# QizhiPei/FABind

Measured on AMD Instinct MI355X. Metric: complexes/sec fwd+bwd (1500p/40l nodes), full IaBNet on the whole graph (pocket model + 4-layer complex model + distance-map head on all nodes / pairs) with the pocket-cls + pocket-centre + coord + distmap + distmap-by-coords + distill losses (BASELINE configs[2] read literally), higher is better.
Workload: dtype bf16

## Files before the change

fabind_amd/_lib.py:

```python
import ctypes
import os

import torch

from . import config as _cfg

_HERE = os.path.dirname(os.path.abspath(__file__))
LIB_PATH = _cfg.knob("FABIND_LIB") or os.path.join(_HERE, "libfabind_hip.so")

ABI_VERSION = 19
DT_F32, DT_BF16 = 0, 1
ACT_NONE, ACT_SILU, ACT_RELU, ACT_SIGMOID, ACT_STORED_DERIV = 0, 1, 2, 3, 4
GEMM_FAM_NT_F32, GEMM_FAM_NT_F32_BF16, GEMM_FAM_NT_BF16, GEMM_FAM_GLDS, GEMM_FAM_PIPE, GEMM_FAM_X3, GEMM_FAM_X3_PRO, GEMM_FAM_PERSIST = range(8)

_vp, _i, _f, _l = ctypes.c_void_p, ctypes.c_int, ctypes.c_float, ctypes.c_long


class GemmArgs(ctypes.Structure):
    _fields_ = [(n, _vp) for n in ("A", "A2", "W", "C", "bias", "R", "r_index", "dotvec", "dot_out", "aux", "groups", "C2")] + \
               [(n, _i) for n in ("M", "N", "K", "K1", "lda", "lda2", "ldw", "ldc", "ldr", "ldaux", "dot_ld",
                                  "a_dtype", "w_dtype", "c_dtype", "aux_dtype", "act_pro", "act_epi", "dact_epi",
                                  "accumulate", "store_preact", "n_groups", "max_m", "max_n", "groups_ext", "epi_fast", "k_splits")] + \
               [("alpha", _f), ("p_drop", _f), ("drop_seed", ctypes.c_uint)] + \
               [(n, _vp) for n in ("row_mu", "row_rs", "col_c", "C16")] + [("ldc16", _i), ("split3", _i), ("r_dtype", _i), ("c2_bf16", _i)]
# ... 103 lines not shown
    "fabind_rowdot_bwd": [_vp, _i, _vp, _i, _vp, _i, _i, _i, _vp, _vp, _vp, _i, _vp],
    "fabind_edge_geom_bwd": [_vp, _vp, _vp, _vp, _vp, _vp, _vp, _vp, _vp, _vp, _i, _i, _i, _vp, _vp, _vp, _vp],
    "fabind_gcl_pre_bwd": [_vp, _i, _i, _vp, _vp, _i, _vp, _vp, _vp, _i, _vp],
    "fabind_gather_dact": [_vp, _i, _vp, _vp, _i, _i, _vp, _i, _i, _i, _vp],
    "fabind_coord_update_bwd": [_vp, _vp, _vp, _i, _i, _f, _vp, _vp, _vp, _vp],
    "fabind_cross_attn_bwd": [_vp, _i, _vp, _i, _vp, _i, _i, _i, _vp, _i, _i, _i, _f, _vp, _vp, _vp, _vp, _vp, _vp, _vp,
                              _vp, _vp, _vp],
    "fabind_pair_bias_cat": [_vp, _i, _vp, _i, _i, _i, _vp, _i, _vp, _i, _vp, _vp, _i, _vp, _i, _vp, _vp],
    "fabind_batched_transpose_pad": [_vp, _i, _vp, _i, _i, _i, _i, _vp, _vp],
    "fabind_node_chain_fwd": [_vp, _i, _vp, _i, _vp, _vp, _vp, _vp, _vp, _vp, _i, _i, _vp, _i, _vp, _i, _vp, _i, _i, _i, _vp],
    "fabind_node_chain_x3_fwd": [_vp, _i, _vp, _i, _vp, _vp, _vp, _vp, _vp, _vp, _vp, _vp, _vp, _vp, _i, _i, _vp, _i, _vp, _i, _vp, _i, _vp, _i, _vp, _i,
                                 _i, _i, _vp],
    "fabind_rows_hadamard_bwd": [_vp, _i, _i, _vp, _i, _i, _vp, _vp, _vp, _i, _vp, _i, _vp],
    "fabind_pair_hadamard_bwd_grid": [_vp, _i, _i, _vp, _i, _i, _vp, _vp, _vp, _vp, _i, _vp, _i, _vp],
    "fabind_pair_hadamard_bwd_rows": [_vp, _i, _i, _vp, _i, _i, _vp, _i, _i, _vp, _vp, _vp, _vp, _i, _vp, _i, _vp, _i, _vp],
    "fabind_pair_hadamard_bwd": [_vp, _i, _i, _vp, _vp, _i, _i, _vp, _vp, _i, _i, _vp, _vp, _i, _vp, _vp, _i, _vp, _vp, _i,
                                 _vp],
    "fabind_inter_attn_bwd": [_vp, _i, _vp, _i, _i, _vp, _vp, _vp, _vp, _vp, _vp, _vp, _vp, _vp, _vp, _vp, _vp, _f, _i,
                              _vp, _vp, _vp, _vp, _vp, _vp, _vp, _vp, _vp, _vp, _i, _vp],
    "fabind_inter_attn_bwd_rows": [_vp, _i, _vp, _i, _i, _vp, _vp, _vp, _vp, _vp, _vp, _vp, _vp, _vp, _vp, _vp, _vp, _f, _i,
                                   _vp, _vp, _vp, _vp, _vp, _vp, _vp, _vp, _vp, _vp, _i, _vp, _i, _i, _vp],
    "fabind_las_step_bwd": [_vp, _vp, _vp, _vp, _vp, _vp, _vp, _vp, _i, _i, _f, _f, _vp, _vp, _vp],
    "fabind_pair_bias_bwd": [_vp, _i, _vp, _i, _i, _vp, _vp, _i, _i, _i, _vp, _vp, _vp, _vp, _vp],
    "fabind_pair_bias_btcat": [_vp, _i, _vp, _vp, _vp, _i, _i, _i, _vp, _i, _i, _vp],
    "fabind_pair_bias_finish": [_vp, _vp, _i, _i, _vp, _vp, _i, _vp, _vp, _l, _vp],
    "fabind_pack_frag_multi": [_vp, _vp, _i, _vp],
    "fabind_lower_bound": [_vp, _i, _vp, _i, _vp, _vp],
    "fabind_pocket_center_fwd": [_vp, _vp, _vp, _vp, _i, _i, _f, _i, _vp, _vp, _vp],
    "fabind_pocket_center_bwd": [_vp, _vp, _vp, _vp, _i, _i, _f, _vp, _vp, _vp, _vp, _vp],
    "fabind_pair_dist_fwd": [_vp, _i, _i, _vp, _vp, _f, _f, _f, _vp, _vp],
    "fabind_pair_dist_bwd": [_vp, _i, _i, _vp, _vp, _vp, _f, _f, _f, _vp, _vp, _vp],
    "fabind_block_hadamard_fwd": [_vp, _i, _i, _vp, _i, _vp, _i, _i, _vp, _i, _vp],
    "fabind_block_hadamard_bwd": [_vp, _i, _i, _vp, _i, _vp, _i, _vp, _i, _i, _vp, _i, _i, _vp, _vp, _i, _vp, _i, _vp],
    "fabind_loss_fwd": [_vp, _vp, _l, _vp, _vp, _vp, _l, _vp, _vp, _i, _vp, _l, _vp, _vp, _l, _f, _f, _f, _f, _f, _f, _vp, _vp, _vp, _vp, _vp, _vp],
    "fabind_loss_bwd": [_vp, _vp, _l, _vp, _vp, _vp, _l, _vp, _vp, _i, _l, _vp, _vp, _l, _f, _f, _f, _f, _f, _f, _vp, _vp, _vp,
                        _vp, _vp, _vp, _vp, _vp, _vp],
    "fabind_layernorm_fwd": [_vp, _vp, _vp, _f, _i, _i, _vp, _vp, _vp, _vp],
    "fabind_layernorm_bwd": [_vp, _vp, _vp, _vp, _vp, _i, _i, _vp, _vp, _vp, _vp],
}

_lib = None


def load():
    global _lib
    if _lib is not None:
        return _lib
    if not os.path.exists(LIB_PATH):
        raise RuntimeError(
            "fabind_amd: %s is missing -- build it with `python -m fabind_amd.build` (hipcc, gfx950). "
            "There is no CPU/eager fallback for the hot path." % LIB_PATH)
    lib = ctypes.CDLL(LIB_PATH)
    lib.fabind_last_error.restype = ctypes.c_char_p
    lib.fabind_abi_version.restype = ctypes.c_int
    got = lib.fabind_abi_version()
    if got != ABI_VERSION:
        raise RuntimeError("fabind_amd: %s has ABI version %d, this binding needs %d -- rebuild with `python -m fabind_amd.build`"
                           % (LIB_PATH, got, ABI_VERSION))
    lib.fabind_sizeof_args.argtypes, lib.fabind_sizeof_args.restype = [ctypes.c_int], ctypes.c_int
    lib.fabind_cross_attn_bwd_scratch.argtypes, lib.fabind_cross_attn_bwd_scratch.restype = [_i, _i, _i], ctypes.c_long
    lib.fabind_pair_bias_cat_parts.argtypes, lib.fabind_pair_bias_cat_parts.restype = [_i, _i], ctypes.c_long
    lib.fabind_cross_attn_fused_bwd_scratch.argtypes, lib.fabind_cross_attn_fused_bwd_scratch.restype = [_i, _i, _i, _i, _i], ctypes.c_long
    lib.fabind_cross_attn_fused_bwd_parts.argtypes, lib.fabind_cross_attn_fused_bwd_parts.restype = [_i, _i], ctypes.c_int
    lib.fabind_pair_bias_finish_parts.argtypes, lib.fabind_pair_bias_finish_parts.restype = [_i], ctypes.c_int
    lib.fabind_loss_blocks.argtypes, lib.fabind_loss_blocks.restype = [_l, _l, _l], ctypes.c_int
    for nm in ("fabind_pair_block_tile", "fabind_pair_block_chunk"):
# ... 58 lines not shown
```

fabind_amd/build.py:

```python
import os
import subprocess
import sys

HERE = os.path.dirname(os.path.abspath(__file__))
CSRC = os.path.join(HERE, "csrc")
INCLUDE = os.path.join(os.path.dirname(HERE), "include")
LIB = os.path.join(HERE, "libfabind_hip.so")
SOURCES = ["capi.hip", "gemm.hip", "graph.hip", "gcl.hip", "fused_edge.hip", "fused_edge_fwd2.hip", "fused_edge_fwd3.hip", "fused_edge_bwd3.hip", "fused_edge_bwd4.hip", "pair_fused.hip", "attn.hip", "inter_attn_rows.hip", "attn_mfma.hip", "norm.hip", "bwd.hip", "post_optim.hip", "node_chain.hip", "heads.hip", "symmetry.hip", "optim.hip"]
HIPCC = os.environ.get("HIPCC", "/opt/rocm/bin/hipcc")
FLAGS = ["--offload-arch=gfx950", "-O3", "-std=c++17", "-fPIC", "-Wno-comment", "-I" + INCLUDE, "-I" + CSRC]


def _stale(out, deps):
    if not os.path.exists(out):
        return True
    t = os.path.getmtime(out)
    return any(os.path.getmtime(d) > t for d in deps)


def build(force=False, verbose=True):
    objs = []
    hdrs = [os.path.join(CSRC, "common.h"), os.path.join(CSRC, "fused_common.h"), os.path.join(INCLUDE, "fabind_hip.h")]
    procs = []
    for src in SOURCES:
        sp = os.path.join(CSRC, src)
        if not os.path.exists(sp):
            raise RuntimeError("fabind_amd.build: source %s is missing" % sp)
        obj = os.path.join(CSRC, src.replace(".hip", ".o"))
        objs.append(obj)
        if force or _stale(obj, [sp] + hdrs):
            cmd = [HIPCC] + FLAGS + ["-c", sp, "-o", obj]
            if verbose:
                print(" ".join(cmd), flush=True)
            procs.append((src, subprocess.Popen(cmd)))
    for src, p in procs:
        if p.wait() != 0:
            raise RuntimeError("hipcc failed on " + src)
    if force or procs or _stale(LIB, objs):
        cmd = [HIPCC, "--offload-arch=gfx950", "-shared", "-fPIC", "-o", LIB] + objs
        if verbose:
            print(" ".join(cmd), flush=True)
# ... 7 lines not shown
```

fabind_amd/models/model.py:

```python
import random

import torch
import torch.nn as nn
import torch.nn.functional as F
from torch.nn import Linear

from .. import kernels as K
from .. import ops
from ..utils.utils import get_keepNode_tensor, gumbel_softmax_no_random
from .att_model import EfficientMCAttModel


class Transition_diff_out_dim(nn.Module):

    def __init__(self, embedding_channels=256, out_channels=256, n=4):
        super().__init__()
        self.layernorm = nn.LayerNorm(embedding_channels)
        self.linear1 = Linear(embedding_channels, n * embedding_channels)
        self.linear2 = Linear(n * embedding_channels, out_channels)
        torch.nn.init.xavier_uniform_(self.linear1.weight, gain=0.001)
        torch.nn.init.xavier_uniform_(self.linear2.weight, gain=0.001)

    def forward(self, z):
        shp = z.shape
# ... 252 lines not shown
        start = _offsets(reps)
        j = torch.arange(pi.shape[0], device=dev) - start[pi]
        ci = _offsets(ncnt)[pocket_batch][pi] + j
        kn = torch.stack([kcnt, ncnt]).tolist()
        return _Pairs(pi, ci, ops.PairBlocks(kn[0], kn[1], dev))

    def _complex_and_heads(self, data, g, plan=None):
        scale = self.coordinate_scale
        cb = data['compound'].batch
        if plan:
            Xn, Xl, cidx, pidx = plan['Xn'], plan['Xl'], plan['cidx'], plan['pidx']
        else:
            Xn = self.normalize_coord(g['X'].unsqueeze(-2)).float()
            Xl = self.normalize_coord(g['XL'].unsqueeze(-2)).float()
            seg1 = g['segment'].bool() if not g['segment'].is_floating_point() else g['segment'] > 0.5
            cidx = torch.nonzero(~seg1 & ~g['is_global']).squeeze(1)
            pidx = torch.nonzero(seg1 & ~g['is_global']).squeeze(1)
        Xo, Ho = self.complex_model(Xn, g['H'], batch_id=g['batch'], segment_id=g['segment'], mask=g['mask'],
                                    is_global=g['is_global'], compound_edge_index=g['c2c'], LAS_edge_index=g['LAS'],
                                    batched_complex_coord_LAS=Xl, LAS_mask=None)
        coords_n = ops.take_unique_rows(Xo, cidx).squeeze(-2)
        return Ho, cidx, pidx, coords_n

    def _dist_heads(self, data, g, Ho, cidx, pidx, coords_n):
        cb = data['compound'].batch
        pairs = g.get('pairs')
        if pairs is None:
            B = int(cb[-1].item()) + 1
            pairs = self._pair_lists(g['pocket_batch'], cb, torch.bincount(g['pocket_batch'], minlength=B), torch.bincount(cb, minlength=B))
        pi, ci = pairs
        ln = ops.layernorm(ops.take_unique_rows(Ho, torch.cat([pidx, cidx])), self.layernorm.weight, self.layernorm.bias, self.layernorm.eps)
        npk = pidx.shape[0]
        blocks = getattr(pairs, 'blocks', None)
        hd = ops.rows_hadamard(ln, pi, npk + ci, a_sorted=True, blocks=blocks, n_a=npk)
        wd = ops.mm_dtype()
        part = ops.linear_rowdot(hd, self.distmap_mlp[0].weight.to(wd), self.distmap_mlp[0].bias,
                                 self.distmap_mlp[2].weight[0].contiguous(), act_epi=K.ACT_RELU)
        y_pred = (part.sum(1) + self.distmap_mlp[2].bias).sigmoid() * 10
        xp = self.normalize_coord(g['pocket_xyz']).float()
        if blocks is not None and coords_n.is_cuda:
            y_by = ops.pair_dist(xp, coords_n, blocks, scale=self.coordinate_scale, lo=0.0, hi=10.0)
        else:
            y_by = self.unnormalize_coord((xp[pi] - ops.take_rows_few(coords_n, ci)).norm(dim=-1)).clamp(0, 10)
        return y_pred, y_by

    def forward(self, data, stage=1, train=False, plan=None):
        cb = data['compound'].batch
        if plan is not None:
            self._adopt_plan(plan, cb.device)
        if plan is not None:
            keep_idx = plan['keep_idx']
        else:
            keep_idx = torch.nonzero(data['pocket'].keepNode).squeeze(1) if (stage == 1 or self.pocket_pred_model.training) else None
        head = self._pocket_head(data, plan)
        training = self.pocket_pred_model.training
        center = self._soft_center(head['logits'], head['mask'], head['xyz'], noise=training)
        pocket_cls = torch.zeros_like(head['mask'], dtype=data.pocket_idx.dtype)
        pocket_cls[head['pb'], head['loc']] = data.pocket_idx
        if training:
            dist = torch.norm(data.coords_center - center, p=2, dim=-1).mean(dim=-1)
            final_stage = 2 if (dist < self.args.center_dist_threshold and random.random() < self.stage_prob) else 1
        else:
            final_stage = stage
        if final_stage == 2:
            c2 = center
            if self.args.local_eval or (self.args.train_pred_pocket_noise and train):
                c2 = center + self.args.train_pred_pocket_noise * (2 * torch.rand_like(center) - 1)
            g = self._stage2(data, head, c2)
        else:
            cx = data['complex']
            pemb = ops.take_unique_rows(head['p_out'], keep_idx if keep_idx is not None else torch.nonzero(data['pocket'].keepNode).squeeze(1))
# ... 62 lines not shown
```

fabind_amd/ops.py:

```python
import ctypes

import numpy as np
import torch

from . import config as _cfg
from . import kernels as K
from ._lib import GemmArgs, check, dt_code, load, ptr, stream


def act_dtype():
    return torch.float32 if _cfg.fp32_storage() else torch.bfloat16


def mm_dtype():
    return torch.float32 if _cfg.fp32_storage() else torch.bfloat16


def _needs_grad(*ts):
    return torch.is_grad_enabled() and any(torch.is_tensor(t) and t.requires_grad for t in ts)


def needs_grad(*ts):
    return _needs_grad(*ts)

# ... 1828 lines not shown
        ctx.save_for_backward(coords, y_pred, y_by, logits, center, coords_true, dis_map, cls, center_true, out)
        ctx.w, ctx.cls_dt = w, cls_dt
        return loss, terms

    @staticmethod
    def backward(ctx, g_loss, g_terms):
        coords, y_pred, y_by, logits, center, coords_true, dis_map, cls, center_true, out = ctx.saved_tensors
        w = ctx.w
        need = ctx.needs_input_grad
        d = [torch.empty_like(t) if need[i] else None for i, t in enumerate((coords, y_pred, y_by, logits, center))]
        gl = None if g_loss is None else g_loss.contiguous().float()
        gt = None if g_terms is None else g_terms.contiguous().float()
        check(load().fabind_loss_bwd(ptr(coords), ptr(coords_true), coords.numel(), ptr(y_pred), ptr(y_by), ptr(dis_map), y_pred.numel(),
                                     ptr(logits), ptr(cls), ctx.cls_dt, logits.numel(), ptr(center), ptr(center_true), center.numel(),
                                     w['coord'], w['pair'], w['distill'], w['cls'], w['center'], w['delta'], ptr(out), ptr(gl), ptr(gt),
                                     ptr(d[0]), ptr(d[1]), ptr(d[2]), ptr(d[3]), ptr(d[4]), stream()), "fabind_loss_bwd")
        return d[0], d[1], d[2], d[3], d[4], None, None, None, None, None, None


def six_term_loss(coords, y_pred, y_by, logits, center, coords_true, dis_map, pocket_cls, p_mask, center_true, w):
    f = lambda t: t.float().contiguous()
    cls = pocket_cls.contiguous()
    if cls.dtype not in _CLS_DT:
        cls = cls.float()
    m8 = p_mask.contiguous().view(torch.uint8) if p_mask.dtype == torch.bool else p_mask.to(torch.uint8).contiguous()
    w = {k: float(v) for k, v in w.items()}
    loss, terms = _SixTermLoss.apply(f(coords), f(y_pred), f(y_by), f(logits), f(center), f(coords_true), f(dis_map), cls, m8,
                                     f(center_true), w)
    tt = terms.unbind(0)
    return loss, {n: tt[i] for i, n in enumerate(LOSS_TERM_NAMES)}


_PAIRBLOCK = np.dtype([("pair_off", np.int64), ("P", np.int32), ("C", np.int32), ("p_row0", np.int32), ("c_row0", np.int32),
                       ("tile0", np.int32), ("pad", np.int32)])


class PairBlocks:

    def __init__(self, kcnt, ncnt, dev):
        from .param_pack import _upload
        kc, nc = np.asarray(kcnt, dtype=np.int64), np.asarray(ncnt, dtype=np.int64)
        B = kc.shape[0]
        tp, ch = load().fabind_pair_block_tile(), load().fabind_pair_block_chunk()
        tiles = (kc + tp - 1) // tp
        d = np.zeros(B, dtype=_PAIRBLOCK)
        d["pair_off"] = np.cumsum(kc * nc) - kc * nc
        d["P"], d["C"] = kc, nc
        d["p_row0"], d["c_row0"] = np.cumsum(kc) - kc, np.cumsum(nc) - nc
        d["tile0"] = np.cumsum(tiles) - tiles
        self.B, self.n_tiles, self.n_pairs = int(B), int(tiles.sum()), int((kc * nc).sum())
        self.max_C, self.n_prows, self.n_crows = int(nc.max()) if B else 0, int(kc.sum()), int(nc.sum())
        self.nchunk_max = (self.max_C + ch - 1) // ch
        self.chunk = ch
        row_b = np.repeat(np.arange(B, dtype=np.int32), nc)
        raw = np.concatenate([d.view(np.uint8), row_b.view(np.uint8)]) if B else np.zeros(0, dtype=np.uint8)
        self.buf = _upload(raw, dev) if raw.shape[0] else None
        self.desc_bytes = d.view(np.uint8).shape[0]

    def tensors(self):
        return [self.buf] if self.buf is not None else []

    @property
    def desc_ptr(self):
        return self.buf.data_ptr()

    @property
    def row_b_ptr(self):
        return self.buf.data_ptr() + self.desc_bytes


class _PairDist(torch.autograd.Function):
    @staticmethod
    def forward(ctx, xp, xc, blocks, scale, lo, hi):
        y = torch.empty(blocks.n_pairs, dtype=torch.float32, device=xc.device)
        check(load().fabind_pair_dist_fwd(blocks.desc_ptr, blocks.B, blocks.n_tiles, ptr(xp), ptr(xc), scale, lo, hi, ptr(y), stream()),
              "fabind_pair_dist_fwd")
        ctx.save_for_backward(xp, xc)
        ctx.blocks, ctx.k = blocks, (scale, lo, hi)
        return y

    @staticmethod
    def backward(ctx, dy):
        xp, xc = ctx.saved_tensors
        bl = ctx.blocks
        part = torch.empty((bl.B, 8, bl.max_C, 3), dtype=torch.float32, device=xc.device)
        dxc = torch.empty_like(xc)
        check(load().fabind_pair_dist_bwd(bl.desc_ptr, bl.B, bl.max_C, ptr(xp), ptr(xc), ptr(dy.contiguous().float()), ctx.k[0], ctx.k[1],
                                          ctx.k[2], ptr(part), ptr(dxc), stream()), "fabind_pair_dist_bwd")
        return None, dxc, None, None, None, None


def pair_dist(xp, xc, blocks, scale=1.0, lo=0.0, hi=10.0):
    assert not xp.requires_grad, "pair_dist: the pocket coordinates are data"
    xp, xc = xp.float().contiguous(), xc.float().contiguous()
    assert xp.shape[0] == blocks.n_prows and xc.shape[0] == blocks.n_crows
    return _PairDist.apply(xp, xc, blocks, float(scale), float(lo), float(hi))
```

include/fabind_hip.h:

```cpp
#ifndef FABIND_HIP_H
#define FABIND_HIP_H

#include <stdint.h>

#ifdef __cplusplus
extern "C" {
#endif

#ifndef __HIP_PLATFORM_AMD__
typedef struct ihipStream_t* hipStream_t;
#endif

const char* fabind_last_error(void);
#define FABIND_ABI_VERSION 19
int fabind_abi_version(void);
int fabind_sizeof_args(int which);

typedef struct FabindGemmArgs {
    const void* A;
    const void* A2;
    const void* W;
    void* C;
    const float* bias;
    const void* R;
// ... 240 lines not shown
int fabind_las_step(const float* x, const float* x0, const int* las_i, const int* las_j, const int* las_off,
                    const int* node_off, const int* c_cnt, int B, int max_n, float step, float clampv, float* x_out,
                    unsigned char* pass_mask, hipStream_t stream);

int fabind_pocket_center_fwd(const float* logits, const uint8_t* mask, const float* xyz, const float* noise, int B, int L,
                             float tau, int hard, float* center, float* wsum, hipStream_t stream);
int fabind_pocket_center_bwd(const float* logits, const uint8_t* mask, const float* xyz, const float* noise, int B, int L,
                             float tau, const float* center, const float* wsum, const float* dcenter, float* dlogits,
                             hipStream_t stream);

int fabind_loss_blocks(long n_pair, long n_coord, long n_cls);
int fabind_loss_fwd(const float* coords, const float* coords_true, long n_coord, const float* y_pred, const float* y_by,
                    const float* dis_map, long n_pair, const float* logits, const void* cls, int cls_dt, const uint8_t* mask,
                    long n_cls, const float* center, const float* center_true, long n_center, float w_coord, float w_pair,
                    float w_distill, float w_cls, float w_center, float delta, float* part, unsigned* ticket, float* out,
                    float* loss_out, float* terms_out, hipStream_t stream);
int fabind_loss_bwd(const float* coords, const float* coords_true, long n_coord, const float* y_pred, const float* y_by,
                    const float* dis_map, long n_pair, const float* logits, const void* cls, int cls_dt, long n_cls,
                    const float* center, const float* center_true, long n_center, float w_coord, float w_pair, float w_distill,
                    float w_cls, float w_center, float delta, const float* fwd_out, const float* g_loss, const float* g_terms,
                    float* d_coords, float* d_y_pred, float* d_y_by, float* d_logits, float* d_center, hipStream_t stream);

int fabind_pair_block_tile(void);
int fabind_pair_block_chunk(void);
int fabind_pair_dist_fwd(const void* desc, int B, int n_tiles, const float* xp, const float* xc, float scale, float lo, float hi,
                         float* y, hipStream_t stream);
int fabind_pair_dist_bwd(const void* desc, int B, int max_C, const float* xp, const float* xc, const float* dy, float scale, float lo,
                         float hi, float* part, float* dxc, hipStream_t stream);
int fabind_block_hadamard_fwd(const void* desc, int B, int n_tiles, const float* tp, int ldtp, const float* tc, int ldtc, int W, void* out,
                              int ldo, hipStream_t stream);
int fabind_block_hadamard_bwd(const void* desc, int B, int n_tiles, const void* dout, int ldo, const float* tp, int ldtp,
                              const float* tc, int ldtc, int W, const int* row_b, int n_crows, int nchunk_max, float* part,
                              float* dtp, int lddp, float* dtc, int lddc, hipStream_t stream);

int fabind_select_rows(const float* x, const float* z, const uint8_t* mask, int n, int width, float* x_out,
                       hipStream_t stream);

int fabind_row_stats(const void* x, int x_dt, int ldx, float eps, int R, int C, float* mu, float* rs, hipStream_t stream);

int fabind_layernorm_rows(const void* x, int x_dt, int ldx, const float* w, const float* b, float eps, int R, int C, void* y,
                          int y_dt, int ldy, int pad_to, hipStream_t stream);
int fabind_edge_ln_concat(const float* h, int ldh, int H, const int* row, const int* col, const float* rhohat, const float* w,
                          const float* b, float eps, int E, void* y, int y_dt, int ldy, int pad_to, hipStream_t stream);

int fabind_edge_lnfold(const void* AB, int ldab, int Kp, int H, const int* row, const int* col, const float* rho,
                       const float* stat, float eps, const float* w_r, const float* c_r, const float* c_c, const float* dvec,
                       int E, void* out, float p_drop, unsigned seed, hipStream_t stream);
int fabind_edge_lnfold_bwd_blocks(int E);
int fabind_edge_lnfold_bwd(const void* AB, int ldab, int Kp, int H, const int* row, const int* col, const float* rho,
                           const float* stat, float eps, const float* w_r, const float* c_r, const float* c_c,
                           const void* out, const void* dout, int E, float p_drop, void* du, float* es,
                           float* drho, float* part, int n_blocks, hipStream_t stream);

int fabind_inter_coord_fold(const void* P, int ldp, int H, const int* col, const float* rho, const float* stat, float q_w,
                            float eps, const float* u, const float* d, const float* w3, int E, float* s_out, float p_drop,
                            unsigned seed, hipStream_t stream);
int fabind_layernorm_rows_bwd(const void* x, int x_dt, int ldx, const float* w, const void* dy, int dy_dt, int lddy, float eps,
                              int R, int C, void* dx, int dx_dt, int lddx, float* dw_part, float* db_part, int nblk, hipStream_t stream);
int fabind_edge_concat(const float* h, int ldh, int H, const int* row, const int* col, const float* rhohat, int E, void* y,
                       int y_dt, int ldy, int pad_to, hipStream_t stream);
int fabind_layernorm_fwd(const float* x, const float* w, const float* b, float eps, int R, int C, float* y, float* mean,
                         float* rstd, hipStream_t stream);
int fabind_layernorm_bwd(const float* x, const float* w, const float* dy, const float* mean, const float* rstd, int R,
                         int C, float* dx, float* dw_part, float* db_part, hipStream_t stream);

int fabind_add(const float* a, const float* b, float* out, long n, hipStream_t stream);
// ... 93 lines not shown
```

Measured before the change: 527.4.

## Fuse distance-map head hadamard, MLP, relu and rowdot into dedicated kernels

Adds a dist_head forward kernel that builds the pocket×compound Hadamard rows in LDS per 64-row tile, runs the 512×512 MFMA GEMM, and applies bias, ReLU and the w2 dot product in the epilogue. It writes per-pair scores, the bf16 hadamard and pre-activations for backward. A matching backward kernel recomputes ReLU gradients, does the transpose GEMM, and reduces the pocket and compound row gradients plus w2 partials, replacing the separate rows_hadamard and linear_rowdot path. The aim is to cut launches and global round trips over the large pair tensor. In exchange it adds a new zf activation buffer, extra bwd partial reductions and eligibility constraints (H=512, bf16).

```diff
diff --git a/fabind_amd/_lib.py b/fabind_amd/_lib.py
--- a/fabind_amd/_lib.py
+++ b/fabind_amd/_lib.py
@@ -159,6 +159,8 @@
     "fabind_pair_dist_bwd": [_vp, _i, _i, _vp, _vp, _vp, _f, _f, _f, _vp, _vp, _vp],
     "fabind_block_hadamard_fwd": [_vp, _i, _i, _vp, _i, _vp, _i, _i, _vp, _i, _vp],
     "fabind_block_hadamard_bwd": [_vp, _i, _i, _vp, _i, _vp, _i, _vp, _i, _i, _vp, _i, _i, _vp, _vp, _i, _vp, _i, _vp],
+    "fabind_dist_head_fwd": [_vp, _i, _i, _i, _vp, _i, _i, _i, _vp, _vp, _vp, _vp, _vp, _vp, _vp],
+    "fabind_dist_head_bwd": [_vp, _i, _i, _i, _vp, _i, _i, _i, _vp, _vp, _vp, _vp, _vp, _vp, _i, _vp, _i, _vp, _vp, _vp],
     "fabind_loss_fwd": [_vp, _vp, _l, _vp, _vp, _vp, _l, _vp, _vp, _i, _vp, _l, _vp, _vp, _l, _f, _f, _f, _f, _f, _f, _vp, _vp, _vp, _vp, _vp, _vp],
     "fabind_loss_bwd": [_vp, _vp, _l, _vp, _vp, _vp, _l, _vp, _vp, _i, _l, _vp, _vp, _l, _f, _f, _f, _f, _f, _f, _vp, _vp, _vp,
                         _vp, _vp, _vp, _vp, _vp, _vp],
diff --git a/fabind_amd/build.py b/fabind_amd/build.py
--- a/fabind_amd/build.py
+++ b/fabind_amd/build.py
@@ -6,7 +6,7 @@
 CSRC = os.path.join(HERE, "csrc")
 INCLUDE = os.path.join(os.path.dirname(HERE), "include")
 LIB = os.path.join(HERE, "libfabind_hip.so")
-SOURCES = ["capi.hip", "gemm.hip", "graph.hip", "gcl.hip", "fused_edge.hip", "fused_edge_fwd2.hip", "fused_edge_fwd3.hip", "fused_edge_bwd3.hip", "fused_edge_bwd4.hip", "pair_fused.hip", "attn.hip", "inter_attn_rows.hip", "attn_mfma.hip", "norm.hip", "bwd.hip", "post_optim.hip", "node_chain.hip", "heads.hip", "symmetry.hip", "optim.hip"]
+SOURCES = ["capi.hip", "gemm.hip", "graph.hip", "gcl.hip", "fused_edge.hip", "fused_edge_fwd2.hip", "fused_edge_fwd3.hip", "fused_edge_bwd3.hip", "fused_edge_bwd4.hip", "pair_fused.hip", "attn.hip", "inter_attn_rows.hip", "attn_mfma.hip", "norm.hip", "bwd.hip", "post_optim.hip", "node_chain.hip", "heads.hip", "dist_head.hip", "symmetry.hip", "optim.hip"]
 HIPCC = os.environ.get("HIPCC", "/opt/rocm/bin/hipcc")
 FLAGS = ["--offload-arch=gfx950", "-O3", "-std=c++17", "-fPIC", "-Wno-comment", "-I" + INCLUDE, "-I" + CSRC]
 
diff --git a/fabind_amd/csrc/dist_head.hip b/fabind_amd/csrc/dist_head.hip
--- /dev/null
+++ b/fabind_amd/csrc/dist_head.hip
@@ -0,0 +1,324 @@
+#include "common.h"
+#include "fabind_hip.h"
+#include "fused_common.h"
+
+namespace {
+
+struct DhBlock { long pair_off; int P, C, p_row0, c_row0, tile0, blk0; };
+
+typedef unsigned dh_u32x2_t __attribute__((ext_vector_type(2)));
+__device__ __forceinline__ void dh_stq(bf16_t* p_, uint32_t a, uint32_t b) { __builtin_nontemporal_store(dh_u32x2_t{a, b}, (dh_u32x2_t*)p_); }
+__device__ __forceinline__ uint2 dh_ldq(const bf16_t* p_) { const dh_u32x2_t v = __builtin_nontemporal_load((const dh_u32x2_t*)p_); return make_uint2(v.x, v.y); }
+__device__ __forceinline__ fe_f2 dh_relu(const fe_f2 z) { return fe_f2{fmaxf(z.x, 0.f), fmaxf(z.y, 0.f)}; }
+
+template <int H, bool SAVE>
+__global__ __launch_bounds__(H, 2) void dist_head_fwd_kernel(const DhBlock* __restrict__ desc, const float* __restrict__ ln, int ld, int n_a,
+                                                             const bf16_t* __restrict__ W1p, const float* __restrict__ b1,
+                                                             const float* __restrict__ w2, float* __restrict__ s_out, bf16_t* hd, bf16_t* zf) {
+    constexpr int BM = FE_BM, MI = BM / 16;
+    constexpr int NW = H / 64;
+    constexpr int CH = H / 8;
+    constexpr int EPW = 64 / CH;
+    constexpr int EPI = NW * EPW;
+    constexpr int NIT = BM / EPI;
+    constexpr int SWZ = 15;
+    extern __shared__ __attribute__((aligned(16))) unsigned char smem[];
+    bf16_t* sX = (bf16_t*)smem;
+    float* sDot = (float*)(sX + BM * H);
+    const DhBlock d = desc[blockIdx.y];
+    const int i0 = (int)blockIdx.x * BM;
+    if (i0 >= d.P) return;
+    const int nr = min(BM, d.P - i0), C = d.C;
+    const int tid = threadIdx.x, lane = tid & 63, wave = tid >> 6;
+    const int fr = lane & 15, cq = lane >> 4;
+    const int sub = lane / CH, ch = lane % CH;
+    const int fcol = wave * 64 + cq * 4;
+
+    float pr[NIT][8];
+#pragma unroll
+    for (int u = 0; u < NIT; ++u) {
+        const int e = u * EPI + wave * EPW + sub;
+        float4 a = make_float4(0.f, 0.f, 0.f, 0.f), b = a;
+        if (e < nr) {
+            const float* src = ln + (size_t)(d.p_row0 + i0 + e) * ld + ch * 8;
+            a = *(const float4*)src; b = *(const float4*)(src + 4);
+        }
+        pr[u][0] = a.x; pr[u][1] = a.y; pr[u][2] = a.z; pr[u][3] = a.w; pr[u][4] = b.x; pr[u][5] = b.y; pr[u][6] = b.z; pr[u][7] = b.w;
+    }
+    const float* lc = ln + (size_t)(n_a + d.c_row0) * ld + ch * 8;
+    const long pair0 = d.pair_off + (long)i0 * C;
+    const __amdgpu_buffer_rsrc_t rs_hd = fe_rsrc(SAVE ? (void*)(hd + (size_t)pair0 * H) : (void*)s_out, SAVE ? (unsigned)nr * C * H * 2 : 0u);
+
+    for (int j = 0; j < C; ++j) {
+        {
+            const float4 c0 = *(const float4*)(lc + (size_t)j * ld), c1 = *(const float4*)(lc + (size_t)j * ld + 4);
+            const float cv[8] = {c0.x, c0.y, c0.z, c0.w, c1.x, c1.y, c1.z, c1.w};
+#pragma unroll
+            for (int u = 0; u < NIT; ++u) {
+                const int e = u * EPI + wave * EPW + sub;
+                float f[8];
+#pragma unroll
+                for (int k = 0; k < 8; ++k) f[k] = pr[u][k] * cv[k];
+                const uint4 v = pack8(f);
+                *(uint4*)&sX[e * H + ((ch ^ (e & SWZ)) * 8)] = v;
+                if constexpr (SAVE)
+                    __builtin_amdgcn_raw_buffer_store_b128(fe_u32x4_t{v.x, v.y, v.z, v.w}, rs_hd, (int)(((unsigned)(e * C + j) * H + ch * 8) * 2), 0,  2);
+            }
+        }
+        __syncthreads();
+
+        f32x4_t acc[MI][4];
+        fe_zero(acc);
+        fe_gemm_rolled<H, MI, true, SWZ>(sX, W1p, wave, lane, acc);
+        {
+            bf16_t* zb = zf + (((size_t)(d.blk0 + (int)blockIdx.x * C + j) * NW + wave) * (MI * 4) * 64 + lane) * 4;
+            fe_f2 da[MI], db[MI];
+#pragma unroll
+            for (int i = 0; i < MI; ++i) { da[i] = fe_f2{0.f, 0.f}; db[i] = da[i]; }
+#pragma unroll
+            for (int jj = 0; jj < 4; ++jj) {
+                const float4 bq = *(const float4*)(b1 + fcol + jj * 16), wq = *(const float4*)(w2 + fcol + jj * 16);
+                const fe_f2 b01 = fe_f2{bq.x, bq.y}, b23 = fe_f2{bq.z, bq.w}, w01 = fe_f2{wq.x, wq.y}, w23 = fe_f2{wq.z, wq.w};
+#pragma unroll
+                for (int i = 0; i < MI; ++i) {
+                    const fe_f2 z01 = fe_f2{acc[i][jj][0], acc[i][jj][1]} + b01, z23 = fe_f2{acc[i][jj][2], acc[i][jj][3]} + b23;
+                    da[i] += dh_relu(z01) * w01;
+                    db[i] += dh_relu(z23) * w23;
+                    if constexpr (SAVE) dh_stq(zb + (size_t)((i * 4 + jj) * 256), fe3_pack(z01), fe3_pack(z23));
+                }
+                __builtin_amdgcn_sched_barrier(0);
+            }
+            float* sd = sDot + (j & 1) * NW * BM + wave * BM;
+#pragma unroll
+            for (int i = 0; i < MI; ++i) {
+                float t = (da[i].x + da[i].y) + (db[i].x + db[i].y);
+                t += __shfl_xor(t, 16, 64);
+                t += __shfl_xor(t, 32, 64);
+                if (cq == 0) sd[i * 16 + fr] = t;
+            }
+        }
+        __syncthreads();
+        if (tid < nr) {
+            const float* sd = sDot + (j & 1) * NW * BM;
+            float s = 0.f;
+#pragma unroll
+            for (int w = 0; w < NW; ++w) s += sd[w * BM + tid];
+            s_out[pair0 + (long)tid * C + j] = s;
+        }
+    }
+}
+
+template <int H>
+__global__ __launch_bounds__(H, 2) void dist_head_bwd_kernel(const DhBlock* __restrict__ desc, const float* __restrict__ ln, int ld, int n_a,
+                                                             const bf16_t* __restrict__ W1Tp, const float* __restrict__ w2,
+                                                             const float* __restrict__ ds, const bf16_t* __restrict__ zf, bf16_t* dz,
+                                                             float* dln, int lddl, float* __restrict__ part, float* __restrict__ w2part) {
+    constexpr int BM = FE_BM, MI = BM / 16;
+    constexpr int NW = H / 64;
+    constexpr int CH = H / 8;
+    constexpr int SWZ = 15;
+    extern __shared__ __attribute__((aligned(16))) unsigned char smem[];
+    bf16_t* sX = (bf16_t*)smem;
+    const int tid = threadIdx.x, lane = tid & 63, wave = tid >> 6;
+    const size_t wg = (size_t)blockIdx.y * gridDim.x + blockIdx.x;
+    const DhBlock d = desc[blockIdx.y];
+    const int i0 = (int)blockIdx.x * BM;
+    if (i0 >= d.P) { w2part[wg * H + tid] = 0.f; return; }
+    const int nr = min(BM, d.P - i0), C = d.C;
+    const int fr = lane & 15, cq = lane >> 4;
+    const int fcol = wave * 64 + cq * 4;
+    const long pair0 = d.pair_off + (long)i0 * C;
+    const __amdgpu_buffer_rsrc_t rs_dz = fe_rsrc(dz + (size_t)pair0 * H, (unsigned)nr * C * H * 2);
+    const __amdgpu_buffer_rsrc_t rs_ds = fe_rsrc(const_cast<float*>(ds) + pair0, (unsigned)nr * C * 4);
+    const __amdgpu_buffer_rsrc_t rs_p = fe_rsrc(const_cast<float*>(ln) + (size_t)(d.p_row0 + i0) * ld, (unsigned)nr * ld * 4);
+    const __amdgpu_buffer_rsrc_t rs_c = fe_rsrc(const_cast<float*>(ln) + (size_t)(n_a + d.c_row0) * ld, (unsigned)C * ld * 4);
+    const __amdgpu_buffer_rsrc_t rs_w2 = fe_rsrc(const_cast<float*>(w2), (unsigned)H * 4);
+#define DH_OPAQUE(v_) asm volatile("" : "+v"(v_))
+
+    f32x4_t dp[MI][4];
+    fe_zero(dp);
+    fe_f2 a3a[4], a3b[4];
+#pragma unroll
+    for (int jj = 0; jj < 4; ++jj) { a3a[jj] = fe_f2{0.f, 0.f}; a3b[jj] = a3a[jj]; }
+
+    for (int j = 0; j < C; ++j) {
+        const size_t blk = (size_t)(d.blk0 + (int)blockIdx.x * C + j);
+        int lz = 0;
+        asm volatile("" : "+s"(lz));
+        const bf16_t* W1Tj = W1Tp + lz;
+        {
+            int ln_ = lane;
+            DH_OPAQUE(ln_);
+            const int fr_ = ln_ & 15, cq_ = ln_ >> 4;
+            const int cx_ = (wave * 8 + (cq_ >> 1)) ^ fr_, lb_ = fr_ * H + (cq_ & 1) * 4;
+            const __amdgpu_buffer_rsrc_t rs_z = fe_rsrc(const_cast<bf16_t*>(zf) + blk * (size_t)(BM * H), (unsigned)BM * H * 2);
+            const unsigned zoff = (unsigned)(wave * (MI * 4) * 64 + ln_) * 8;
+            uint2 zq[4][MI];
+#pragma unroll
+            for (int jj = 0; jj < 4; ++jj)
+#pragma unroll
+                for (int i = 0; i < MI; ++i) {
+                    const dh_u32x2_t v = __builtin_amdgcn_raw_buffer_load_b64(rs_z, (int)zoff, (i * 4 + jj) * 512,  2);
+                    zq[jj][i] = make_uint2(v.x, v.y);
+                }
+            float dsr[MI];
+#pragma unroll
+            for (int i = 0; i < MI; ++i) {
+                const int row = i * 16 + fr_;
+                const float v = __uint_as_float(__builtin_amdgcn_raw_buffer_load_b32(rs_ds, min(row, nr - 1) * C * 4, j * 4, 0));
+                dsr[i] = row < nr ? v : 0.f;
+            }
+            const unsigned woff = (unsigned)(wave * 64 + cq_ * 4) * 4;
+            __syncthreads();
+#pragma unroll
+            for (int jj = 0; jj < 4; ++jj) {
+                const uint4 wu = fe3_bload16(rs_w2, woff, (unsigned)(jj * 64));
+                const fe_f2 w01 = fe_f2{__uint_as_float(wu.x), __uint_as_float(wu.y)}, w23 = fe_f2{__uint_as_float(wu.z), __uint_as_float(wu.w)};
+#pragma unroll
+                for (int i = 0; i < MI; ++i) {
+                    const fe_f2 z01 = fe3_unpack(zq[jj][i].x), z23 = fe3_unpack(zq[jj][i].y);
+                    const fe_f2 g01 = fe_f2{z01.x > 0.f ? w01.x : 0.f, z01.y > 0.f ? w01.y : 0.f} * dsr[i];
+                    const fe_f2 g23 = fe_f2{z23.x > 0.f ? w23.x : 0.f, z23.y > 0.f ? w23.y : 0.f} * dsr[i];
+                    a3a[jj] += dh_relu(z01) * dsr[i];
+                    a3b[jj] += dh_relu(z23) * dsr[i];
+                    *(uint2*)&sX[lb_ + i * 16 * H + ((cx_ ^ (jj * 2)) * 8)] = make_uint2(fe3_pack(g01), fe3_pack(g23));
+                }
+                asm volatile("" : "+v"(a3a[jj]), "+v"(a3b[jj]));
+                __builtin_amdgcn_sched_barrier(0);
+            }
+        }
+        __syncthreads();
+
+        {
+            int t_ = tid;
+            DH_OPAQUE(t_);
+#pragma unroll
+            for (int it = 0; it < BM * CH / H; ++it) {
+                const int q = t_ + it * H;
+                const int rw = q / CH, c8 = q % CH;
+                const uint4 v = *(const uint4*)&sX[rw * H + ((c8 ^ (rw & SWZ)) * 8)];
+                __builtin_amdgcn_raw_buffer_store_b128(fe_u32x4_t{v.x, v.y, v.z, v.w}, rs_dz, (int)(((unsigned)(rw * C + j) * H + c8 * 8) * 2), 0,  2);
+            }
+        }
+        __builtin_amdgcn_sched_barrier(0);
+        f32x4_t acc[MI][4];
+        fe_zero(acc);
+        fe_gemm_rolled<H, MI, true, SWZ>(sX, W1Tj, wave, lane, acc);
+        __builtin_amdgcn_sched_barrier(0);
+
+        {
+            int ln_ = lane;
+            DH_OPAQUE(ln_);
+            const int fr_ = ln_ & 15, cq_ = ln_ >> 4;
+            const unsigned coff = (unsigned)(wave * 64 + cq_ * 4) * 4;
+            const __amdgpu_buffer_rsrc_t rs_part = fe_rsrc(part + blk * H, (unsigned)H * 4);
+#pragma unroll
+            for (int jj = 0; jj < 4; ++jj) {
+                const uint4 cu = fe3_bload16(rs_c, coff, (unsigned)((j * ld + jj * 16) * 4));
+                uint4 pu[MI];
+#pragma unroll
+                for (int i = 0; i < MI; ++i) pu[i] = fe3_bload16(rs_p, (unsigned)(min(i * 16 + fr_, nr - 1) * ld) * 4 + coff, (unsigned)(jj * 64));
+                const float c4[4] = {__uint_as_float(cu.x), __uint_as_float(cu.y), __uint_as_float(cu.z), __uint_as_float(cu.w)};
+                float t[4] = {0.f, 0.f, 0.f, 0.f};
+#pragma unroll
+                for (int i = 0; i < MI; ++i) {
+                    const f32x4_t a = acc[i][jj];
+                    const float p4[4] = {__uint_as_float(pu[i].x), __uint_as_float(pu[i].y), __uint_as_float(pu[i].z), __uint_as_float(pu[i].w)};
+#pragma unroll
+                    for (int r = 0; r < 4; ++r) { dp[i][jj][r] += a[r] * c4[r]; t[r] += a[r] * p4[r]; }
+                }
+#pragma unroll
+                for (int r = 0; r < 4; ++r) t[r] = fe3_row16_sum(t[r]);
+                if (fr_ == 0) fe3_bstore16(rs_part, coff, (unsigned)(jj * 64), make_uint4(__float_as_uint(t[0]), __float_as_uint(t[1]), __float_as_uint(t[2]), __float_as_uint(t[3])));
+                __builtin_amdgcn_sched_barrier(0);
+            }
+        }
+    }
+#undef DH_OPAQUE
+
+#pragma unroll
+    for (int i = 0; i < MI; ++i) {
+        if (i * 16 + fr < nr) {
+            float* o = dln + (size_t)(d.p_row0 + i0 + i * 16 + fr) * lddl + fcol;
+#pragma unroll
+            for (int jj = 0; jj < 4; ++jj) *(float4*)(o + jj * 16) = make_float4(dp[i][jj][0], dp[i][jj][1], dp[i][jj][2], dp[i][jj][3]);
+        }
+    }
+#pragma unroll
+    for (int jj = 0; jj < 4; ++jj) {
+        float t[4] = {a3a[jj].x, a3a[jj].y, a3b[jj].x, a3b[jj].y};
+#pragma unroll
+        for (int r = 0; r < 4; ++r) t[r] = fe3_row16_sum(t[r]);
+        if (fr == 0) *(float4*)(w2part + wg * H + fcol + jj * 16) = make_float4(t[0], t[1], t[2], t[3]);
+    }
+}
+
+__global__ __launch_bounds__(256) void dist_head_reduce_kernel(const DhBlock* __restrict__ desc, const int* __restrict__ row_b, int H,
+                                                               const float* __restrict__ part, float* dtc, int lddc) {
+    const int r = blockIdx.x;
+    const DhBlock d = desc[row_b[r]];
+    const int j = r - d.c_row0, nt = (d.P + FE_BM - 1) / FE_BM;
+    for (int c = threadIdx.x; c < H; c += 256) {
+        float v = 0.f;
+        for (int t = 0; t < nt; ++t) v += part[(size_t)(d.blk0 + t * d.C + j) * H + c];
+        dtc[(size_t)r * lddc + c] = v;
+    }
+}
+
+constexpr size_t dh_lds(int H, bool fwd) { return (size_t)FE_BM * H * 2 + (fwd ? (size_t)2 * (H / 64) * FE_BM * sizeof(float) : 0); }
+
+}
+
+extern "C" int fabind_dist_head_fwd(const void* desc, int B, int max_tiles, int max_C, const float* ln, int ld, int n_a, int H, const void* W1p,
+                                    const float* b1, const float* w2, float* s, void* hd, void* zf, hipStream_t stream) {
+    FB_REQUIRE(H == 512, "fabind_dist_head_fwd: H = 512");
+    FB_REQUIRE(desc && ln && W1p && b1 && w2 && s && ((hd != nullptr) == (zf != nullptr)), "fabind_dist_head_fwd: null operand (hd and zf come together)");
+    FB_REQUIRE(ld % 4 == 0 && ((((uintptr_t)ln | (uintptr_t)W1p | (uintptr_t)b1 | (uintptr_t)w2 | (uintptr_t)hd | (uintptr_t)zf) & 15) == 0),
+               "fabind_dist_head_fwd: 16-byte aligned rows");
+    FB_REQUIRE(max_C >= 0 && (uint64_t)max_C * FE_BM * H * 2 < (1ull << 32), "fabind_dist_head_fwd: 64 * max_C * H * 2 bytes must stay below 4 GiB");
+    if (B <= 0 || max_tiles <= 0 || max_C <= 0) return 0;
+    const size_t lds = dh_lds(512, true);
+    static bool set_ = false;
+    if (!set_) {
+        hipError_t e_ = hipFuncSetAttribute((const void*)dist_head_fwd_kernel<512, true>, hipFuncAttributeMaxDynamicSharedMemorySize, (int)lds);
+        if (e_ == hipSuccess) e_ = hipFuncSetAttribute((const void*)dist_head_fwd_kernel<512, false>, hipFuncAttributeMaxDynamicSharedMemorySize, (int)lds);
+        if (e_ != hipSuccess) { fabind_set_error(hipGetErrorString(e_)); return (int)e_; }
+        set_ = true;
+    }
+    if (hd)
+        hipLaunchKernelGGL((dist_head_fwd_kernel<512, true>), dim3(max_tiles, B), dim3(512), lds, stream, (const DhBlock*)desc, ln, ld, n_a,
+                           (const bf16_t*)W1p, b1, w2, s, (bf16_t*)hd, (bf16_t*)zf);
+    else
+        hipLaunchKernelGGL((dist_head_fwd_kernel<512, false>), dim3(max_tiles, B), dim3(512), lds, stream, (const DhBlock*)desc, ln, ld, n_a,
+                           (const bf16_t*)W1p, b1, w2, s, (bf16_t*)nullptr, (bf16_t*)nullptr);
+    FB_CHECK_LAUNCH();
+    return 0;
+}
+
+extern "C" int fabind_dist_head_bwd(const void* desc, int B, int max_tiles, int max_C, const float* ln, int ld, int n_a, int H, const void* W1Tp,
+                                    const float* w2, const float* ds, const void* zf, void* dz, float* dln, int lddl, const int* row_b,
+                                    int n_crows, float* part, float* w2part, hipStream_t stream) {
+    FB_REQUIRE(H == 512, "fabind_dist_head_bwd: H = 512");
+    FB_REQUIRE(desc && ln && W1Tp && w2 && ds && zf && dz && dln && row_b && part && w2part, "fabind_dist_head_bwd: null operand");
+    FB_REQUIRE(ld % 4 == 0 && lddl % 4 == 0 &&
+               ((((uintptr_t)ln | (uintptr_t)W1Tp | (uintptr_t)w2 | (uintptr_t)zf | (uintptr_t)dz | (uintptr_t)dln | (uintptr_t)part | (uintptr_t)w2part) & 15) == 0),
+               "fabind_dist_head_bwd: 16-byte aligned rows");
+    FB_REQUIRE(max_C >= 0 && (uint64_t)max_C * FE_BM * H * 2 < (1ull << 32), "fabind_dist_head_bwd: 64 * max_C * H * 2 bytes must stay below 4 GiB");
+    if (B <= 0 || max_tiles <= 0 || max_C <= 0) return 0;
+    const size_t lds = dh_lds(512, false);
+    static bool set_ = false;
+    if (!set_) {
+        const hipError_t e_ = hipFuncSetAttribute((const void*)dist_head_bwd_kernel<512>, hipFuncAttributeMaxDynamicSharedMemorySize, (int)lds);
+        if (e_ != hipSuccess) { fabind_set_error(hipGetErrorString(e_)); return (int)e_; }
+        set_ = true;
+    }
+    hipLaunchKernelGGL((dist_head_bwd_kernel<512>), dim3(max_tiles, B), dim3(512), lds, stream, (const DhBlock*)desc, ln, ld, n_a,
+                       (const bf16_t*)W1Tp, w2, ds, (const bf16_t*)zf, (bf16_t*)dz, dln, lddl, part, w2part);
+    FB_CHECK_LAUNCH();
+    if (n_crows > 0) {
+        hipLaunchKernelGGL(dist_head_reduce_kernel, dim3(n_crows), dim3(256), 0, stream, (const DhBlock*)desc, row_b, H, part,
+                           dln + (size_t)n_a * lddl, lddl);
+        FB_CHECK_LAUNCH();
+    }
+    return 0;
+}
diff --git a/fabind_amd/models/model.py b/fabind_amd/models/model.py
--- a/fabind_amd/models/model.py
+++ b/fabind_amd/models/model.py
@@ -308,11 +308,10 @@
         ln = ops.layernorm(ops.take_unique_rows(Ho, torch.cat([pidx, cidx])), self.layernorm.weight, self.layernorm.bias, self.layernorm.eps)
         npk = pidx.shape[0]
         blocks = getattr(pairs, 'blocks', None)
-        hd = ops.rows_hadamard(ln, pi, npk + ci, a_sorted=True, blocks=blocks, n_a=npk)
         wd = ops.mm_dtype()
-        part = ops.linear_rowdot(hd, self.distmap_mlp[0].weight.to(wd), self.distmap_mlp[0].bias,
-                                 self.distmap_mlp[2].weight[0].contiguous(), act_epi=K.ACT_RELU)
-        y_pred = (part.sum(1) + self.distmap_mlp[2].bias).sigmoid() * 10
+        s = ops.dist_head(ln, pi, npk + ci, self.distmap_mlp[0].weight.to(wd), self.distmap_mlp[0].bias,
+                          self.distmap_mlp[2].weight[0].contiguous(), blocks=blocks, n_a=npk)
+        y_pred = (s + self.distmap_mlp[2].bias).sigmoid() * 10
         xp = self.normalize_coord(g['pocket_xyz']).float()
         if blocks is not None and coords_n.is_cuda:
             y_by = ops.pair_dist(xp, coords_n, blocks, scale=self.coordinate_scale, lo=0.0, hi=10.0)
diff --git a/fabind_amd/ops.py b/fabind_amd/ops.py
--- a/fabind_amd/ops.py
+++ b/fabind_amd/ops.py
@@ -1884,7 +1884,8 @@
 
 
 _PAIRBLOCK = np.dtype([("pair_off", np.int64), ("P", np.int32), ("C", np.int32), ("p_row0", np.int32), ("c_row0", np.int32),
-                       ("tile0", np.int32), ("pad", np.int32)])
+                       ("tile0", np.int32), ("blk0", np.int32)])
+DIST_HEAD_TILE = 64
 
 
 class PairBlocks:
@@ -1900,6 +1901,10 @@
         d["P"], d["C"] = kc, nc
         d["p_row0"], d["c_row0"] = np.cumsum(kc) - kc, np.cumsum(nc) - nc
         d["tile0"] = np.cumsum(tiles) - tiles
+        t64 = (kc + DIST_HEAD_TILE - 1) // DIST_HEAD_TILE
+        d["blk0"] = np.cumsum(t64 * nc) - t64 * nc
+        self.n_blk64, self.max_tiles64 = int((t64 * nc).sum()), int(t64.max()) if B else 0
+        self.min_P, self.min_C = (int(kc.min()), int(nc.min())) if B else (0, 0)
         self.B, self.n_tiles, self.n_pairs = int(B), int(tiles.sum()), int((kc * nc).sum())
         self.max_C, self.n_prows, self.n_crows = int(nc.max()) if B else 0, int(kc.sum()), int(nc.sum())
         self.nchunk_max = (self.max_C + ch - 1) // ch
@@ -1921,6 +1926,69 @@
         return self.buf.data_ptr() + self.desc_bytes
 
 
+class _DistHead(torch.autograd.Function):
+
+    @staticmethod
+    def forward(ctx, ln, W1, b1, w2, blocks, n_a):
+        H = ln.shape[1]
+        dev = ln.device
+        W1p, W1Tp = K.pack_frag_multi([W1, W1.t()])
+        s = torch.empty(blocks.n_pairs, dtype=torch.float32, device=dev)
+        hd = torch.empty((blocks.n_pairs, H), dtype=torch.bfloat16, device=dev)
+        zf = torch.empty(blocks.n_blk64 * DIST_HEAD_TILE * H, dtype=torch.bfloat16, device=dev)
+        K._profiled("fabind_dist_head_fwd H=%d pairs=%d" % (H, blocks.n_pairs), 2.0 * blocks.n_pairs * H * H,
+                    lambda: check(load().fabind_dist_head_fwd(blocks.desc_ptr, blocks.B, blocks.max_tiles64, blocks.max_C, ptr(ln), ln.stride(0), n_a,
+                                                              H, ptr(W1p), ptr(b1), ptr(w2), ptr(s), ptr(hd), ptr(zf), stream()), "fabind_dist_head_fwd"),
+                    nbytes=2.0 * (hd.numel() + zf.numel()))
+        ctx.blocks, ctx.n_a = blocks, n_a
+        ctx.save_for_backward(ln, W1, w2, hd, zf, W1Tp)
+        return s
+
+    @staticmethod
+    def backward(ctx, ds):
+        ln, W1, w2, hd, zf, W1Tp = ctx.saved_tensors
+        bl, H, dev = ctx.blocks, ln.shape[1], ln.device
+        ds = ds.contiguous().float()
+        dz = torch.empty_like(hd)
+        dln = torch.empty_like(ln)
+        part = torch.empty((bl.n_blk64, H), dtype=torch.float32, device=dev)
+        w2part = torch.empty((bl.B * bl.max_tiles64, H), dtype=torch.float32, device=dev)
+        K._profiled("fabind_dist_head_bwd H=%d pairs=%d" % (H, bl.n_pairs), 2.0 * bl.n_pairs * H * H,
+                    lambda: check(load().fabind_dist_head_bwd(bl.desc_ptr, bl.B, bl.max_tiles64, bl.max_C, ptr(ln), ln.stride(0), ctx.n_a, H, ptr(W1Tp),
+                                                              ptr(w2), ptr(ds), ptr(zf), ptr(dz), ptr(dln), dln.stride(0), bl.row_b_ptr, bl.n_crows,
+                                                              ptr(part), ptr(w2part), stream()), "fabind_dist_head_bwd"),
+                    nbytes=2.0 * (dz.numel() + zf.numel()))
+        dW1, db1 = _weight_grad(dz, hd, K.ACT_NONE, None, W1.dtype, want_db=True, W=W1)
+        return dln, dW1, db1, K.colsum(w2part), None, None
+
+
+DIST_HEAD_FUSED = True
+
+
+def dist_head_eligible(ln, W1, b1, w2, blocks, n_a):
+    return (DIST_HEAD_FUSED and blocks is not None and _cfg.get_precision() == "bf16" and ln.is_cuda and ln.dtype == torch.float32 and ln.dim() == 2
+            and ln.shape[1] == 512 and ln.is_contiguous() and ln.data_ptr() % 16 == 0 and W1.dtype == torch.bfloat16 and tuple(W1.shape) == (512, 512)
+            and b1 is not None and b1.dtype == torch.float32 and w2.dtype == torch.float32 and b1.is_contiguous() and w2.is_contiguous()
+            and n_a == blocks.n_prows and ln.shape[0] == blocks.n_prows + blocks.n_crows and blocks.B > 0 and blocks.min_P > 0 and blocks.min_C > 0
+            and blocks.max_C < 32768)
+
+
+def dist_head(ln, idx_a, idx_b, W1, b1, w2, blocks=None, n_a=0):
+    if not dist_head_eligible(ln, W1, b1, w2, blocks, n_a):
+        hd = rows_hadamard(ln, idx_a, idx_b, a_sorted=True, blocks=blocks, n_a=n_a)
+        return linear_rowdot(hd, W1, b1, w2, act_epi=K.ACT_RELU).sum(1)
+    if _needs_grad(ln, W1, b1, w2):
+        K.tn_hook(W1, b1)
+        return _DistHead.apply(ln, W1, b1, w2, blocks, n_a)
+    H = ln.shape[1]
+    W1p, = K.pack_frag_multi([W1])
+    s = torch.empty(blocks.n_pairs, dtype=torch.float32, device=ln.device)
+    K._profiled("fabind_dist_head_fwd H=%d pairs=%d" % (H, blocks.n_pairs), 2.0 * blocks.n_pairs * H * H,
+                lambda: check(load().fabind_dist_head_fwd(blocks.desc_ptr, blocks.B, blocks.max_tiles64, blocks.max_C, ptr(ln), ln.stride(0), n_a, H,
+                                                          ptr(W1p), ptr(b1), ptr(w2), ptr(s), None, None, stream()), "fabind_dist_head_fwd"))
+    return s
+
+
 class _PairDist(torch.autograd.Function):
     @staticmethod
     def forward(ctx, xp, xc, blocks, scale, lo, hi):
diff --git a/include/fabind_hip.h b/include/fabind_hip.h
--- a/include/fabind_hip.h
+++ b/include/fabind_hip.h
@@ -296,6 +296,12 @@
 int fabind_block_hadamard_bwd(const void* desc, int B, int n_tiles, const void* dout, int ldo, const float* tp, int ldtp,
                               const float* tc, int ldtc, int W, const int* row_b, int n_crows, int nchunk_max, float* part,
                               float* dtp, int lddp, float* dtc, int lddc, hipStream_t stream);
+
+int fabind_dist_head_fwd(const void* desc, int B, int max_tiles, int max_C, const float* ln, int ld, int n_a, int H, const void* W1p,
+                         const float* b1, const float* w2, float* s, void* hd, void* zf, hipStream_t stream);
+int fabind_dist_head_bwd(const void* desc, int B, int max_tiles, int max_C, const float* ln, int ld, int n_a, int H, const void* W1Tp,
+                         const float* w2, const float* ds, const void* zf, void* dz, float* dln, int lddl, const int* row_b, int n_crows,
+                         float* part, float* w2part, hipStream_t stream);
 
 int fabind_select_rows(const float* x, const float* z, const uint8_t* mask, int n, int width, float* x_out,
                        hipStream_t stream);
```

After: 554.1 (median of 6 runs). 1.05x the previous value.
